# edawson/rkmh

Hardware: AMD Instinct MI355X
Metric: reads classified/sec (higher is better)
Workload: dtype u64; 1 GPU; stream (C2): 1000000 synthetic 150 bp reads per GPU vs data/all_pave_ref.fa (182 refs), k=16 s=1000; reads_per_gpu=1000000, read_len=150, k=16, sketch_size=1000, references=182, parallelism=reads sharded over 1 rank(s); ref sketches RCCL-broadcast once

## Files before the change

rkmh_amd/csrc/rk_kmer.hip:

```cpp
#include "rk_kernels.hpp"

#include <cstdlib>
#include <type_traits>

namespace rk {

namespace {

constexpr int KW = 64;
constexpr int KM_MAX_T = 8;
constexpr int KM_MQ = 32;
constexpr int KM_CH = 2;
constexpr int KM_QCAP = 64 + 4 * KW;
constexpr int KM_LDS_SMALL = 5120;
constexpr int KM_LDS_BIG = 20480;
constexpr int KM_WAVES = 8;

enum { CM_DENSE8 = 0, CM_DENSE16 = 1, CM_SPARSE = 2 };

struct KmerGeom {
    int32_t T;
    int32_t cwords;
    int32_t dset;
    int32_t xcd;
    int32_t nmin_cap;
    int32_t L;
    int32_t gpr[KM_MAX_KS];
    uint32_t magic[KM_MAX_KS];
};

typedef uint32_t u32x4 __attribute__((ext_vector_type(4)));
struct __attribute__((packed, aligned(1))) km_pair1 { uint32_t x, y; };
struct __attribute__((packed, aligned(4))) km_pair4 { uint32_t x, y; };

template <int NQ>
struct KmLds {
    static constexpr int PK = 0;
    static constexpr int INV = PK + NQ * 64 + 2;
    static constexpr int Q = INV + NQ * 32 + 2;
    static constexpr int MQ = Q + KM_QCAP;
    static constexpr int RI = MQ + 2 * KM_MQ;
    static constexpr int NZ = RI + 4 * (KM_MAX_T + 1);
    static constexpr int BEST = NZ + KM_MAX_T;
    static constexpr int FLAGS = BEST + KM_MAX_T;
    static constexpr int NWT = FLAGS + KM_MAX_T;
    static constexpr int FAM = NWT + KM_MAX_T;
    static constexpr int FAMF = FAM + 4 * KM_MAX_T;
    static constexpr int CNT = FAMF + KM_MAX_T;
    static_assert(RI % 4 == 0, "rinfo is read with 16-byte LDS loads");
    static_assert(CNT % 4 == 0, "the multisets are cleared with 16-byte LDS stores");
};
inline size_t km_lds_bytes(const KmerGeom& g, int nq) {
    return ((size_t)(nq == 1 ? KmLds<1>::CNT : KmLds<2>::CNT) + (size_t)g.T * (size_t)(g.cwords + g.dset)) * 4;
}

__device__ __forceinline__ void wave_sync() {
    __builtin_amdgcn_fence(__ATOMIC_RELEASE, "wavefront");
    __builtin_amdgcn_wave_barrier();
    __builtin_amdgcn_fence(__ATOMIC_ACQUIRE, "wavefront");
}
template <int CTRL>
__device__ __forceinline__ int dpp_i32(int v) { return __builtin_amdgcn_update_dpp(v, v, CTRL, 0xf, 0xf, false); }
__device__ __forceinline__ int row_max_i32(int v) {
    int t;
    t = dpp_i32<0xB1>(v); v = t > v ? t : v;
    t = dpp_i32<0x4E>(v); v = t > v ? t : v;
    t = dpp_i32<0x141>(v); v = t > v ? t : v;
    t = dpp_i32<0x140>(v); v = t > v ? t : v;
    return v;
}
__device__ __forceinline__ int half_row_max_i32(int v) {
    int t;
    t = dpp_i32<0xB1>(v); v = t > v ? t : v;
    t = dpp_i32<0x4E>(v); v = t > v ? t : v;
    t = dpp_i32<0x141>(v); v = t > v ? t : v;
    return v;
}

__device__ __forceinline__ uint32_t km_pack4_hi(uint32_t x, uint32_t& mism) {
    const uint32_t c = (x >> 1) & 0x03030303u;
    mism |= (x & 0xDFDFDFDFu) ^ __builtin_amdgcn_perm(0x47544341u, 0x47544341u, c);
    return c * 0x01041040u;
}
__device__ __forceinline__ uint32_t km_pack16(const u32x4& v, uint32_t& mism) {
    const uint32_t m0 = km_pack4_hi(v.x, mism), m1 = km_pack4_hi(v.y, mism), m2 = km_pack4_hi(v.z, mism), m3 = km_pack4_hi(v.w, mism);
    const uint32_t lo = __builtin_amdgcn_perm(m1, m0, 0x0c0c0703u);
    const uint32_t hi = __builtin_amdgcn_perm(m3, m2, 0x07030c0cu);
    return lo | hi;
}
__device__ __forceinline__ uint32_t km_nonzero4(uint32_t m) {
    const uint32_t y = (m | ((m & 0x7f7f7f7fu) + 0x7f7f7f7fu)) & 0x80808080u;
    return ((y >> 7) * 0x01020408u) >> 24;
}

template <int CMODE>
__device__ __forceinline__ uint32_t km_field_max(uint32_t x) {
    if constexpr (CMODE == CM_DENSE8) {
        const uint32_t m01 = max(x & 0xFFu, (x >> 8) & 0xFFu), m23 = max((x >> 16) & 0xFFu, x >> 24);
        return max(m01, m23);
    } else return max(x & 0xFFFFu, x >> 16);
}

template <int KT, int NQ, int CMODE, bool BIG, bool FAM>
__global__ __launch_bounds__(KW, BIG ? 2 : KM_WAVES) void k_classify_kmer(const uint8_t* __restrict__ bases, const uint32_t* __restrict__ offs,
                                                                              uint32_t nreads, int S, RefIndex ix, KmerSets ksets,
                                                                              int32_t* __restrict__ out4, DevPolicy pol, KmerGeom geo) {
    static_assert(KT == 0 || KT == 32 || (KT >= 4 && KT <= 16), "a k-mer packs into 32 bits; the core is the (k-3)-mer");
    constexpr bool WIDE = KT == 32;
    using L = KmLds<NQ>;
    __shared__ __attribute__((aligned(16))) uint32_t smem[(BIG ? KM_LDS_BIG : KM_LDS_SMALL) / 4];
    constexpr uint32_t PAD_P = NQ * 1024;
    constexpr uint32_t clg = CMODE == CM_DENSE8 ? 2 : 1, cbits = 32u >> clg, cmask = (1u << cbits) - 1u;
    uint32_t* const pk = smem + L::PK;
    uint32_t* const inv = smem + L::INV;
    uint32_t* const q = smem + L::Q;
    uint32_t* const mq = smem + L::MQ;
    uint4* const rinfo = reinterpret_cast<uint4*>(smem + L::RI);
    uint32_t* const nzero = smem + L::NZ;
    uint32_t* const best = smem + L::BEST;
    uint32_t* const flags = smem + L::FLAGS;
    uint32_t* const nwtot = smem + L::NWT;
    uint32_t* const fam = smem + L::FAM;
    uint32_t* const famf = smem + L::FAMF;
    uint32_t* const cnt = smem + L::CNT;
    const int T = geo.T;
    const uint32_t CW = (uint32_t)geo.cwords, DS = (uint32_t)geo.dset;
    uint32_t* const dset = cnt + (uint32_t)T * CW;
    const uint32_t ds_shift = 32u - (uint32_t)__builtin_ctz(DS);
    const int lane = threadIdx.x;

    for (uint32_t i = lane; i < ((uint32_t)T * CW) >> 2; i += KW) reinterpret_cast<uint4*>(cnt)[i] = make_uint4(0u, 0u, 0u, 0u);
    const uint32_t ntiles = (nreads + (uint32_t)T - 1) / (uint32_t)T;
    const uintptr_t gb = reinterpret_cast<uintptr_t>(bases);
    const uintptr_t safe_hi = (gb + (uintptr_t)offs[nreads] + 4u) & ~(uintptr_t)3;

    auto tile_reads = [&](uint32_t tl) -> int {
        const uint32_t r = tl * (uint32_t)T;
        return (int)((nreads - r) < (uint32_t)T ? (nreads - r) : (uint32_t)T);
    };
    auto load_offsets = [&](uint32_t tl, uint32_t& a_, uint32_t& b_, uint32_t& o_) {
        const uint32_t r = tl * (uint32_t)T;
        const int n = tile_reads(tl);
        a_ = offs[r];
        b_ = offs[r + (uint32_t)n];
        o_ = offs[r + (uint32_t)(lane <= n ? lane : n)];
    };
    u32x4 pf[NQ];
    auto fetch_tile = [&](uint32_t a_, uint32_t b_) {
        const uintptr_t first = gb + a_;
        const uintptr_t base16 = first & ~(uintptr_t)15;
        const uint32_t nbytes = (uint32_t)(first - base16) + (b_ - a_);
        uint32_t nq = (nbytes + 15u) >> 4;
        if (nq > (uint32_t)(NQ * KW)) nq = NQ * KW;
        const bool safe = base16 >= gb && base16 + 16u * (uintptr_t)nq <= safe_hi;
#pragma unroll
        for (int r = 0; r < NQ; ++r) {
            const uint32_t qi = (uint32_t)r * KW + (uint32_t)lane;
            u32x4 v = {0u, 0u, 0u, 0u};
            if (qi < nq) {
                const uintptr_t qa = base16 + 16u * (uintptr_t)qi;
                if (safe) {
                    typedef const u32x4 __attribute__((address_space(1))) * gq_t;
                    v = __builtin_nontemporal_load((gq_t)qa);
                }
                else {
                    uint32_t d[4];
#pragma unroll
                    for (int j = 0; j < 4; ++j) {
                        const uintptr_t da = qa + 4u * (uintptr_t)j;
                        d[j] = (da >= gb && da + 4u <= safe_hi) ? *reinterpret_cast<const uint32_t*>(da) : 0u;
                    }
                    v.x = d[0]; v.y = d[1]; v.z = d[2]; v.w = d[3];
                }
            }
            pf[r] = v;
        }
    };

    uint32_t tile = blockIdx.x;
    if (geo.xcd) { const uint32_t per = (gridDim.x + 7u) >> 3; tile = (blockIdx.x & 7u) * per + (blockIdx.x >> 3); }
    if (tile >= ntiles) return;
    uint32_t cur_a = 0, cur_b = 0, cur_o = 0;
    load_offsets(tile, cur_a, cur_b, cur_o);
    fetch_tile(cur_a, cur_b);
    {
        const uint32_t r0 = tile * (uint32_t)T;
        const uint32_t ta = (uint32_t)__builtin_amdgcn_readfirstlane((int)cur_a);
        const uint32_t tb = (uint32_t)__builtin_amdgcn_readfirstlane((int)cur_b);
        const uint32_t mis = (uint32_t)((gb + ta) & 15u);
        const uint32_t nbytes = mis + (tb - ta);
        const uint32_t o_next = (uint32_t)__shfl_down((int)cur_o, 1);
        const uint32_t len = o_next - cur_o;
        int Tn = tile_reads(tile);
        uint32_t nq = (nbytes + 15u) >> 4;
        if (nbytes > (uint32_t)(NQ * 1024)) {
            const int Tn0 = Tn;
            Tn = __popcll(__ballot(lane < Tn0 && o_next - ta + mis <= (uint32_t)(NQ * 1024)));
            if (lane >= Tn && lane < Tn0) reinterpret_cast<int4*>(out4)[r0 + lane] = make_int4(-2, 0, 0, 0);
            nq = NQ * KW;
        }

        constexpr int NKC = KT ? 1 : KM_MAX_KS;
        const int NK = KT ? 1 : ksets.n;
        uint32_t nw_all = 0;
        if (lane < Tn) {
#pragma unroll
            for (int j = 0; j < NKC; ++j) if (j < NK) nw_all += (uint32_t)num_windows((int)len, WIDE ? (int)ix.kpk : (KT ? KT : ksets.k[j]), pol.drop_last_window);
        }
        if constexpr (FAM) { if (lane < 4 * KM_MAX_T) fam[lane] = 0; }
        if (lane < KM_MAX_T) {
            nzero[lane] = 0; best[lane] = 0; nwtot[lane] = nw_all;
            if constexpr (FAM) famf[lane] = 0;
            flags[lane] = nw_all > (CMODE == CM_SPARSE ? 0x7FFu : cmask) ? 1u : 0u;
        }
        const uint32_t ulen = (uint32_t)__builtin_amdgcn_readfirstlane((int)len);
        const bool same_len = __ballot(lane < Tn && len != ulen) == 0ull;
        uint32_t mism = 0;
#pragma unroll
        for (int r = 0; r < NQ; ++r) {
            const uint32_t qi = (uint32_t)r * KW + (uint32_t)lane;
            uint32_t m = 0;
            pk[qi] = km_pack16(pf[r], m);
            if (qi < nq) mism |= m;
        }
        if (lane < 2) pk[NQ * KW + lane] = 0;
        const bool has_invalid = __ballot(mism != 0u) != 0ull;
        if (has_invalid) {
#pragma unroll
            for (int r = 0; r < NQ; ++r) {
                const uint32_t qi = (uint32_t)r * KW + (uint32_t)lane;
                uint32_t m0 = 0, m1 = 0, m2 = 0, m3 = 0;
                km_pack4_hi(pf[r].x, m0); km_pack4_hi(pf[r].y, m1); km_pack4_hi(pf[r].z, m2); km_pack4_hi(pf[r].w, m3);
                const uint32_t b16 = km_nonzero4(m0) | (km_nonzero4(m1) << 4) | (km_nonzero4(m2) << 8) | (km_nonzero4(m3) << 12);
                reinterpret_cast<uint16_t*>(inv)[qi] = (uint16_t)(qi < nq ? b16 : 0u);
            }
            if (lane < 2) inv[NQ * 32 + lane] = 0;
        }
        for (int kk = 0; kk < NK; ++kk) {
        const int k = WIDE ? (int)ix.kpk : (KT ? KT : ksets.k[kk]);
        const uint32_t KMASK = (WIDE || k == 16) ? 0xffffffffu : ((1u << (2 * k)) - 1u);
        const uint32_t CMASK = WIDE ? 0xffffffffu : (1u << (2 * (k - 3))) - 1u;
        const uint64_t KMASK64 = WIDE ? (1ull << (2 * k)) - 1ull : 0ull, CMASK64 = WIDE ? (1ull << (2 * (k - 3))) - 1ull : 0ull;
        const uint32_t KBITS = (1u << k) - 1u;
        const uint4* const kf4p = KT ? ix.kf4 : ksets.kf4[kk];
        const uint4* const km1p = KT ? ix.km1 : ksets.km1[kk];
        const uint32_t* const km1v = KT ? ix.km1_vals : ksets.km1_vals[kk];
        const uint32_t kf4_n = KT ? ix.kf4_n : ksets.kf4_n[kk], km1_b = KT ? ix.km1_b : ksets.km1_b[kk];
        wave_sync();
        uint32_t nw = 0, ng = 0;
        if (lane < Tn) { nw = (uint32_t)num_windows((int)len, k, pol.drop_last_window); ng = (nw + 3u) >> 2; }
        uint32_t gs = ng;
        gs += (uint32_t)__builtin_amdgcn_update_dpp(0, (int)gs, 0x111, 0xf, 0xf, true);
        gs += (uint32_t)__builtin_amdgcn_update_dpp(0, (int)gs, 0x112, 0xf, 0xf, true);
        gs += (uint32_t)__builtin_amdgcn_update_dpp(0, (int)gs, 0x114, 0xf, 0xf, true);
        const uint32_t NG = (uint32_t)__builtin_amdgcn_readlane((int)gs, KM_MAX_T - 1);
        if (lane <= KM_MAX_T) rinfo[lane] = make_uint4(cur_o - ta + mis, nw, gs - ng, 0u);
        {
            uint4* d4 = reinterpret_cast<uint4*>(dset);
            for (uint32_t i = lane; i < ((uint32_t)Tn * DS) >> 2; i += KW) d4[i] = make_uint4(0u, 0u, 0u, 0u);
        }
        wave_sync();

        const uint32_t nw_u = (uint32_t)num_windows((int)ulen, k, pol.drop_last_window), gpr_u = (nw_u + 3u) >> 2;
        const bool uniform = same_len && gpr_u >= 2u;
        uint32_t magic = 0;
        if (uniform) magic = ulen == (uint32_t)geo.L ? geo.magic[kk] : (uint32_t)__builtin_amdgcn_readfirstlane((int)(0xFFFFFFFFu / gpr_u + 1u));
        uint32_t magic_v = magic, dlen_v = ulen - 4u * gpr_u;
        asm volatile("" : "+v"(magic_v), "+v"(dlen_v));

        auto count_posting = [&](uint32_t t, uint32_t crow_b, uint32_t ref) -> uint32_t {
            uint32_t* crow = reinterpret_cast<uint32_t*>(reinterpret_cast<uint8_t*>(cnt) + crow_b);
            const uint32_t M1 = CW - 1u, key = ref + 1u;
            uint32_t idx = ((ref * 0x9E3779B1u) >> 16) & M1, probe = 0, c = 0;
            for (; probe <= M1; ++probe) {
                const uint32_t old = atomicCAS(&crow[idx], 0u, (key << 11) | 1u);
                if (old == 0u) { c = 1u; break; }
                if ((old >> 11) == key) { c = (atomicAdd(&crow[idx], 1u) & 0x7FFu) + 1u; break; }
                idx = (idx + 1u) & M1;
            }
            if (probe > M1) { flags[t] = 1; return 0u; }
            return (c << 16) + (0xFFFFu - ref);
        };
        auto add_posting = [&](uint32_t t, uint32_t crow_b, uint32_t ref) {
            if constexpr (CMODE == CM_SPARSE) {
                const uint32_t v = count_posting(t, crow_b, ref);
                if (v) atomicMax(&best[t], v);
            } else {
                const uint32_t sh = (ref << (5 - clg)) & (32u - cbits);
                const uint32_t woff = (ref >> clg) << 2;
                atomicAdd(reinterpret_cast<uint32_t*>(reinterpret_cast<uint8_t*>(cnt) + crow_b + woff), 1u << sh);
            }
        };
        uint32_t mqn = 0;
        auto process_mq = [&]() {
            wave_sync();
            const uint32_t g = (uint32_t)lane >> 4, sl = (uint32_t)lane & 15u;
            auto walk = [&](uint32_t tr, const uint32_t* lp, uint32_t hdr, const km_pair4& pm0) {
                const uint32_t t = tr & 0xFFu, n = hdr & 0xFFFFFFu, base = FAM ? hdr >> 24 : 0u;
                if (base) {
                    if ((tr >> 8) != 0u) return;
                    if (sl == 0) { atomicAdd(&fam[4u * t + ((base - 1u) >> 1)], 1u << (16u * ((base - 1u) & 1u))); famf[t] = 1u; }
                    for (uint32_t c0 = 0; c0 < n; c0 += 16) {
                        const uint32_t c = c0 + sl;
                        if (c < n) {
                            km_pair4 pm = pm0;
                            if (c0) pm = *reinterpret_cast<const km_pair4*>(lp + 1 + 2 * c);
                            const uint32_t sh = (pm.x << (5 - clg)) & (32u - cbits), woff = (pm.x >> clg) << 2;
                            atomicAdd(reinterpret_cast<uint32_t*>(reinterpret_cast<uint8_t*>(cnt) + __umul24(t, CW * 4u) + woff), (pm.y >> 31) ? 0u - (1u << sh) : 1u << sh);
                        }
                    }
                    return;
                }
                for (uint32_t c0 = 0; c0 < n; c0 += 16) {
                    const uint32_t c = c0 + sl;
                    uint32_t v = 0;
                    if (c < n) {
                        km_pair4 pm = pm0;
                        if (c0) pm = *reinterpret_cast<const km_pair4*>(lp + 1 + 2 * c);
                        if ((tr >> 8) < pm.y) {
                            if constexpr (CMODE == CM_SPARSE) v = count_posting(t, __umul24(t, CW * 4u), pm.x);
                            else add_posting(t, __umul24(t, CW * 4u), pm.x);
                        }
                    }
                    if constexpr (CMODE == CM_SPARSE) {
                        v = (uint32_t)row_max_i32((int)v);
                        if (sl == 0 && v) atomicMax(&best[t], v);
                    }
                }
            };
            uint32_t j = g;
            uint32_t tr = 0, n = 0;
            const uint32_t* lp = ix.kpost;
            km_pair4 pm0{0u, 0u};
            if (j < mqn) { tr = mq[2 * j]; lp = ix.kpost + mq[2 * j + 1]; n = lp[0]; pm0 = *reinterpret_cast<const km_pair4*>(lp + 1 + 2 * sl); }
            while (j < mqn) {
                const uint32_t jn = j + KW / 16;
                uint32_t trn = 0, nn = 0;
                const uint32_t* lpn = ix.kpost;
                km_pair4 pmn{0u, 0u};
                if (jn < mqn) { trn = mq[2 * jn]; lpn = ix.kpost + mq[2 * jn + 1]; nn = lpn[0]; pmn = *reinterpret_cast<const km_pair4*>(lpn + 1 + 2 * sl); }
                walk(tr, lp, n, pm0);
                j = jn; tr = trn; lp = lpn; n = nn; pm0 = pmn;
            }
            wave_sync();
            mqn = 0;
        };
        struct Cand { uint32_t key, t, y, key_hi; uint4 c; };
        const uint32_t km_r = WIDE ? 8u : 2u * (uint32_t)k - km1_b, km_vb1 = 32u - KM1_HB - km_r;
        const uint32_t km_vmask = (1u << (km_vb1 - 1u)) - 1u, km_rmask = (1u << km_r) - 1u, nref = (uint32_t)ix.nref;
        auto wide_probe = [&](const Cand& c, const uint4& b, uint32_t hop, uint3& res, bool& again) {
            const uint32_t want = (hop << KW_TAG) | (c.y & ((1u << KW_TAG) - 1u));
            const uint32_t cells[4] = {b.x, b.y, b.z, b.w};
            res = make_uint3(KW_VID_NONE, 0u, 0u);
#pragma unroll
            for (int q = 0; q < 4; ++q) {
                const uint32_t num = cells[q] & KW_EMPTY;
                if ((cells[q] >> (KW_IDBITS + 1)) == want && num != KW_EMPTY && res.x == KW_VID_NONE) {
                    const uint2 kk = ix.kkeys[num];
                    if (kk.x == c.key && (kk.y & 0xFFu) == c.key_hi) res = make_uint3(kk.y >> 8, 0u, num);
                }
            }
            again = res.x == KW_VID_NONE && ((b.w >> KW_IDBITS) & 1u) != 0u && c.t != 0xFFFFFFFFu;
        };
        auto lookup = [&](uint32_t e, uint32_t qn) -> Cand {
            Cand c;
            uint32_t ent = PAD_P | (8u << 12);
            if (e < qn) ent = q[e];
            const uint32_t P = ent & 4095u, t = ent >> 12;
            const km_pair1 w = *reinterpret_cast<const km_pair1*>(reinterpret_cast<const uint8_t*>(pk) + (P >> 2));
            const uint2 ri = *reinterpret_cast<const uint2*>(&rinfo[t]);
            c.t = P - ri.x < ri.y ? t : 0xFFFFFFFFu;
            if constexpr (WIDE) {
                const uint64_t x = (join64(w.x, w.y) >> ((P & 3u) << 1)) & KMASK64;
                const uint64_t r = packed_revcomp64(x, k);
                const uint64_t key = x < r ? x : r;
                c.key = (uint32_t)key; c.key_hi = (uint32_t)(key >> 32);
                c.y = (uint32_t)(kw_y(key, k) >> (2u * (uint32_t)k - km1_b - KW_TAG));
                c.c = km1p[c.y >> KW_TAG];
                return c;
            }
            const uint32_t x = __builtin_amdgcn_alignbit(w.y, w.x, (P & 3u) << 1) & KMASK;
            const uint32_t r = packed_revcomp(x, k);
            c.key = x < r ? x : r;
            c.key_hi = 0;
            c.y = km1_y(c.key, k);
            c.c = km1p[c.y >> km_r];
            return c;
        };
        auto match_cell = [&](const uint4& b, uint32_t wantsh) -> uint32_t {
            const uint32_t lim = 1u << km_vb1;
            return (b.x ^ wantsh) < lim ? b.x : ((b.y ^ wantsh) < lim ? b.y : ((b.z ^ wantsh) < lim ? b.z : ((b.w ^ wantsh) < lim ? b.w : 0xFFFFFFFFu)));
        };
        auto first_match = [&](const Cand& c, uint32_t& cell, bool& again) {
            cell = match_cell(c.c, (c.y & km_rmask) << km_vb1);
            again = (cell & km_vmask) == km_vmask && ((c.c.w >> (km_vb1 - 1u)) & 1u) != 0u && c.t != 0xFFFFFFFFu;
        };
        auto hop_load = [&](const Cand& c, uint32_t hop, bool again) -> u32x4 {
            u32x4 v = {0u, 0u, 0u, 0u};
            if (again) v = *reinterpret_cast<const u32x4*>(km1p + (((c.y >> km_r) + hop) & ((1u << km1_b) - 1u)));
            return v;
        };
        auto next_match = [&](const Cand& c, uint32_t hop, const u32x4& nv, uint32_t& cell, bool& again) {
            if (again) {
                const uint4 nb = make_uint4(nv.x, nv.y, nv.z, nv.w);
                cell = match_cell(nb, ((c.y & km_rmask) << km_vb1) | (hop << (32u - KM1_HB)));
                again = (cell & km_vmask) == km_vmask && ((nb.w >> (km_vb1 - 1u)) & 1u) != 0u;
            }
        };
        auto apply = [&](const Cand& c, uint32_t cell, uint3 wres = make_uint3(0u, 0u, 0u)) {
            uint32_t vid = cell & km_vmask;
            bool hit = vid != km_vmask && c.t != 0xFFFFFFFFu;
            bool zero = vid == km_vmask - 1u;
            if constexpr (WIDE) {
                vid = wres.x;
                hit = vid != KW_VID_NONE && c.t != 0xFFFFFFFFu;
                zero = vid == KW_VID_ZERO;
                if (hit && !zero && ix.keepkey) { const uint32_t kid = ix.kslots[wres.z]; if (!((ix.keepkey[kid >> 5] >> (kid & 31u)) & 1u)) zero = true; }
            }
            uint32_t val = vid | (1u << 20);
            uint32_t valy = 0, valz = 0, valw = 0;
            if (hit && vid >= nref && !zero) {
                const uint4 vv = *reinterpret_cast<const uint4*>(km1v + 4u * (vid - nref));
                val = vv.x; valy = vv.y; valz = vv.z; valw = vv.w;
                if constexpr (CMODE == CM_SPARSE) { if ((val >> 29) == 7u) val = 0x80000000u | valz; }
            }
            uint32_t rank = 0;
            bool multi = false;
            if (hit) {
                if (zero) atomicAdd(&nzero[c.t], 1u);
                else {
                    uint32_t* ds = dset + c.t * DS;
                    const uint32_t id = (WIDE ? wres.z : c.key) + 1u;
                    uint32_t idx = ((id - 1u) * 0x9E3779B1u) >> ds_shift;
                    uint32_t old = atomicCAS(&ds[idx], 0u, id);
                    uint32_t probes = 1;
                    while (old != 0u && probes < DS) {
                        rank += old == id ? 1u : 0u;
                        idx = (idx + 1u) & (DS - 1u);
                        old = atomicCAS(&ds[idx], 0u, id);
                        ++probes;
                    }
                    if (old != 0u) flags[c.t] = 1;
                    else if (FAM && (val >> 29) == 7u) {
                        if (rank == 0) {
                            const uint32_t base = (val >> 26) & 7u, nex = (val >> 22) & 15u, crow_b = __umul24(c.t, CW * 4u);
                            atomicAdd(&fam[4u * c.t + (base >> 1)], 1u << (16u * (base & 1u)));
                            famf[c.t] = 1u;
                            auto signed_add = [&](uint32_t f) {
                                const uint32_t ref = f & 511u, sh = (ref << (5 - clg)) & (32u - cbits);
                                atomicAdd(reinterpret_cast<uint32_t*>(reinterpret_cast<uint8_t*>(cnt) + crow_b + ((ref >> clg) << 2)), (f & 512u) ? 0u - (1u << sh) : 1u << sh);
                            };
                            if (nex > 0u) signed_add(val & 1023u);
                            if (nex > 1u) signed_add((val >> 10) & 1023u);
                            if (nex > 2u) signed_add(valy & 1023u);
                            if (nex > 3u) signed_add((valy >> 10) & 1023u);
                            if (nex > 4u) signed_add((valy >> 20) & 1023u);
                            if (nex > 5u) signed_add(valw & 1023u);
                            if (nex > 6u) signed_add((valw >> 10) & 1023u);
                            if (nex > 7u) signed_add((valw >> 20) & 1023u);
                        }
                    }
                    else if ((val >> 30) == 3u || !(val >> 31)) {
                        const bool three = (val >> 30) == 3u, two = !three && ((val >> 29) & 3u) != 0u;
                        const uint32_t fw = three ? 9u : 11u;
                        const uint32_t lim = (three || two) ? 1u : ((val >> 20) & 0x1FFu);
                        const uint32_t n = rank >= lim ? 0u : (three ? 3u + ((val >> 27) & 3u) : (two ? 2u : 1u));
                        const uint32_t refs[6] = {__builtin_amdgcn_ubfe(val, 0u, three ? 9u : (two ? 11u : 20u)), __builtin_amdgcn_ubfe(val, fw, fw),
                                                  (val >> 18) & 511u, valy & 511u, (valy >> 9) & 511u, (valy >> 18) & 511u};
                        const uint32_t crow_b = __umul24(c.t, CW * 4u);
#pragma unroll
                        for (uint32_t j = 0; j < 6u; ++j) if (j < n) add_posting(c.t, crow_b, refs[j]);
                    } else multi = true;
                }
            }
            const uint32_t listoff = (CMODE == CM_SPARSE ? valz : val) & 0x3fffffffu;
            uint64_t mm = __ballot(multi);
            while (mm) {
                const uint32_t pos = __builtin_amdgcn_mbcnt_hi((uint32_t)(mm >> 32), __builtin_amdgcn_mbcnt_lo((uint32_t)mm, 0u));
                const uint32_t space = (uint32_t)KM_MQ - mqn;
                if (multi && pos < space) {
                    mq[2 * (mqn + pos)] = c.t | (rank << 8); mq[2 * (mqn + pos) + 1] = listoff;
                    multi = false;
                }
                const uint32_t tot = (uint32_t)__popcll(mm);
                mqn += tot < space ? tot : space;
                if (mqn == (uint32_t)KM_MQ) process_mq();
                mm = __ballot(multi);
            }
        };
        auto drain = [&](uint32_t qn) {
            for (uint32_t e0 = 0; e0 < qn; e0 += 2 * KW) {
                const bool two = e0 + KW < qn;
                const Cand a = lookup(e0 + (uint32_t)lane, qn);
                Cand b{0u, 0xFFFFFFFFu, 0u, 0u, make_uint4(0u, 0u, 0u, 0u)};
                if (two) b = lookup(e0 + KW + (uint32_t)lane, qn);
                if constexpr (WIDE) {
                    uint3 ra, rb = make_uint3(KW_VID_NONE, 0u, 0u);
                    bool ga, gb = false;
                    wide_probe(a, a.c, 0u, ra, ga);
                    if (two) wide_probe(b, b.c, 0u, rb, gb);
                    for (uint32_t hop = 1; hop < (1u << KM1_HB) && __ballot(ga || gb); ++hop) {
                        const uint32_t bm = (1u << km1_b) - 1u;
                        if (ga) { const uint4 nb = km1p[((a.y >> KW_TAG) + hop) & bm]; wide_probe(a, nb, hop, ra, ga); }
                        if (gb) { const uint4 nb = km1p[((b.y >> KW_TAG) + hop) & bm]; wide_probe(b, nb, hop, rb, gb); }
                    }
                    apply(a, 0u, ra);
                    if (two) apply(b, 0u, rb);
                    continue;
                }
                uint32_t ca, cb = 0xFFFFFFFFu;
                bool ga, gb = false;
                first_match(a, ca, ga);
                if (two) first_match(b, cb, gb);
                for (uint32_t hop = 1; hop < (1u << KM1_HB) && __ballot(ga || gb); ++hop) {
                    u32x4 na = hop_load(a, hop, ga), nb = hop_load(b, hop, gb);
                    asm volatile("" : "+v"(na), "+v"(nb));
                    next_match(a, hop, na, ca, ga);
                    next_match(b, hop, nb, cb, gb);
                }
                apply(a, ca);
                if (two) apply(b, cb);
            }
            if (mqn) process_mq();
        };

        const uint32_t nsteps = (NG + KW - 1) / KW;
        const bool qlast = !WIDE && NG != 0u && ((NG - 1u) & (uint32_t)(KW - 1)) < 16u;
        const uint32_t kf4_n16 = kf4_n << 4;
        uint32_t qcount = 0;
        uint32_t step = 0;
        for (;;) {
            uint32_t wl[KM_CH], wh[KM_CH], e0v[KM_CH], fq[KM_CH];
            u32x4 fw[KM_CH];
            bool isqv[KM_CH];
#pragma unroll
            for (int s = 0; s < KM_CH; ++s) {
                const bool isq = qlast && step + (uint32_t)s + 1u == nsteps;
                isqv[s] = isq;
                const uint32_t jq = isq ? (uint32_t)lane & 3u : 0u;
                const uint32_t G = (step + (uint32_t)s) * KW + (isq ? (uint32_t)lane >> 2 : (uint32_t)lane);
                uint32_t t, P0;
                if (uniform) {
                    t = __umulhi(G, magic_v);
                    P0 = __umul24(t, dlen_v) + ((G << 2) + mis);
                } else {
                    t = 0;
#pragma unroll
                    for (int i = 1; i < KM_MAX_T; ++i) t += G >= rinfo[i].z ? 1u : 0u;
                    const uint4 ri = rinfo[t];
                    P0 = ri.x + 4u * (G - ri.z);
                }
                const bool act = G < NG;
                if (!act) { P0 = PAD_P; t = 8u; }
                const km_pair1 w = *reinterpret_cast<const km_pair1*>(reinterpret_cast<const uint8_t*>(pk) + (P0 >> 2));
                const uint32_t sh = (P0 & 3u) << 1;
                wl[s] = __builtin_amdgcn_alignbit(w.y, w.x, sh);
                wh[s] = w.y >> sh;
                uint32_t core = k == 16 ? wl[s] >> 6 : (wl[s] >> 6) & CMASK;
                if constexpr (WIDE) core = kw_fold((join64(wl[s], wh[s]) >> 6) & CMASK64);
                const uint32_t sect_b = __umulhi(core * 0x85EBCA6Bu, kf4_n16) & ~15u;
                e0v[s] = P0 | (t << 12);
                fq[s] = 0u;
                fw[s] = u32x4{0u, 0u, 0u, 0u};
                if (isq) {
                    wl[s] = __builtin_amdgcn_alignbit(wh[s], wl[s], 2u * jq);
                    if (act) e0v[s] += jq;
                    fq[s] = *reinterpret_cast<const uint32_t*>(reinterpret_cast<const uint8_t*>(kf4p) + (sect_b + 4u * jq));
                } else fw[s] = *reinterpret_cast<const u32x4*>(reinterpret_cast<const uint8_t*>(kf4p) + sect_b);
            }
            bool stop = false;
            uint32_t done = 0;
            auto test_step = [&](int s, auto inv_tag, auto nw_tag) {
                constexpr bool INV = decltype(inv_tag)::value;
                constexpr int NW = decltype(nw_tag)::value;
                uint32_t ib = 0, nz = 0, nwt = 0, t_ = 0, o0 = 0;
                bool act = true;
                if constexpr (INV) {
                    const uint32_t P0 = e0v[s] & 4095u;
                    t_ = e0v[s] >> 12;
                    act = t_ != 8u;
                    if (act) {
                        ib = __builtin_amdgcn_alignbit(inv[(P0 >> 5) + 1], inv[P0 >> 5], P0 & 31u);
                        const uint2 ri = *reinterpret_cast<const uint2*>(&rinfo[t_]);
                        nwt = ri.y; o0 = P0 - ri.x;
                    }
                }
#pragma unroll
                for (int j = 0; j < NW; ++j) {
                    uint32_t x = j == 0 ? wl[s] : __builtin_amdgcn_alignbit(wh[s], wl[s], 2 * j);
                    if (k < 16) x &= KMASK;
                    if constexpr (WIDE) x = kw_fold((join64(wl[s], wh[s]) >> (2 * j)) & KMASK64);
                    const uint32_t f = NW == 1 ? fq[s] : (j == 0 ? fw[s].x : (j == 1 ? fw[s].y : (j == 2 ? fw[s].z : fw[s].w)));
                    const uint32_t fb = kf4_bits_dev(x);
                    bool cand = (fb & f) == fb;
                    if constexpr (INV) {
                        if (act && ((ib >> j) & KBITS) != 0u) {
                            cand = false;
                            if (o0 + (uint32_t)j < nwt) ++nz;
                        }
                    }
                    const uint64_t m = __builtin_amdgcn_ballot_w64(cand);
                    if (__builtin_amdgcn_inverse_ballot_w64(m)) {
                        const uint32_t mb = __builtin_amdgcn_mbcnt_hi((uint32_t)(m >> 32), __builtin_amdgcn_mbcnt_lo((uint32_t)m, 0u));
                        *reinterpret_cast<uint32_t*>(reinterpret_cast<uint8_t*>(q) + ((mb << 2) + (qcount << 2))) = e0v[s] + (uint32_t)j;
                    }
                    qcount += (uint32_t)__builtin_popcountll(m);
                }
                if constexpr (INV) { if (nz) atomicAdd(&nzero[t_], nz); }
            };
#pragma unroll
            for (int s = 0; s < KM_CH; ++s) {
                if (step + (uint32_t)s < nsteps && !stop) {
                    if (qcount + 4u * KW > (uint32_t)KM_QCAP) stop = true;
                    else {
                        ++done;
                        if (isqv[s]) {
                            if (has_invalid) test_step(s, std::true_type{}, std::integral_constant<int, 1>{});
                            else test_step(s, std::false_type{}, std::integral_constant<int, 1>{});
                        } else if (has_invalid) test_step(s, std::true_type{}, std::integral_constant<int, 4>{});
                        else test_step(s, std::false_type{}, std::integral_constant<int, 4>{});
                    }
                }
            }
            step += done;
            const bool last = step >= nsteps;
            wave_sync();
            const uint32_t qn = last ? qcount : (qcount & ~(uint32_t)(KW - 1));
            drain(qn);
            wave_sync();
            if (last) break;
            const uint32_t rem = qcount - qn;
            uint32_t ce = 0;
            if ((uint32_t)lane < rem) ce = q[qn + lane];
            wave_sync();
            if ((uint32_t)lane < rem) q[lane] = ce;
            qcount = rem;
            wave_sync();
        }

        }
        wave_sync();

        {
            const int lsh = Tn > 4 ? 3 : 4, LPR = 1 << lsh;
            const int g = lane >> lsh, sl = lane & (LPR - 1);
            for (int t = g; t < Tn; t += KW >> lsh) {
                uint32_t* ct = cnt + (uint32_t)t * CW;
                const int nmins = (int)nwtot[t] - (int)nzero[t];
                const bool reroute = nmins > S || flags[t] != 0;
                if (reroute) {
                    if (sl == 0) reinterpret_cast<int4*>(out4)[r0 + t] = make_int4(-2, 0, 0, 0);
                    continue;
                }
                if constexpr (FAM && CMODE != CM_SPARSE) {
                    if (famf[t]) {
                        for (uint32_t b = 0; b < 8u; ++b) {
                            const uint32_t h = (fam[4u * (uint32_t)t + (b >> 1)] >> (16u * (b & 1u))) & 0xFFFFu;
                            if (h == 0u) continue;
                            const uint32_t start = ix.kbase[2u * b], nm = ix.kbase[2u * b + 1u];
                            for (uint32_t m0 = 0; m0 < nm; m0 += (uint32_t)LPR) {
                                const uint32_t m = m0 + (uint32_t)sl;
                                if (m < nm) {
                                    const uint32_t ref = ix.kbase[start + m];
                                    atomicAdd(&ct[ref >> clg], h << ((ref << (5 - clg)) & (32u - cbits)));
                                }
                            }
                        }
                        __builtin_amdgcn_fence(__ATOMIC_RELEASE, "wavefront");
                        __builtin_amdgcn_fence(__ATOMIC_ACQUIRE, "wavefront");
                    }
                }
                int max_id, max_shared, prev;
                if constexpr (CMODE == CM_SPARSE) {
                    const uint32_t bk = best[t];
                    max_id = bk ? (int)(0xFFFFu - (bk & 0xFFFFu)) : 0;
                    max_shared = (int)(bk >> 16);
                    prev = max_id > 0 ? 0 : -1;
                    for (uint32_t w = sl; w < CW; w += LPR) {
                        const uint32_t x = ct[w];
                        const int r_ = (int)(x >> 11) - 1, cj = (int)(x & 0x7FFu);
                        if (x != 0u && r_ < max_id && cj > prev) prev = cj;
                    }
                } else {
                    const uint32_t nwl = (CW + (uint32_t)LPR - 1u) >> lsh, wbase = (uint32_t)sl * nwl;
                    uint32_t lmax = 0, lpre = 0, lfirst = wbase;
                    for (uint32_t i = 0; i < nwl; ++i) {
                        const uint32_t w = wbase + i;
                        const uint32_t m = km_field_max<CMODE>(ct[w < CW ? w : CW - 1u]);
                        if (m > lmax) { lpre = lmax; lmax = m; lfirst = w; }
                    }
                    const uint32_t lkey = (lmax << 8) | (255u - lfirst);
                    const uint32_t km = (uint32_t)(LPR == 16 ? row_max_i32((int)lkey) : half_row_max_i32((int)lkey));
                    const uint32_t M = km >> 8, wb = 255u - (km & 255u);
                    const uint32_t xb = ct[wb];
                    const uint32_t ones = CMODE == CM_DENSE8 ? 0x01010101u : 0x00010001u;
                    const uint32_t y = xb ^ (M * ones);
                    const uint32_t z = (y - ones) & ~y & (ones << (cbits - 1u));
                    const uint32_t qf = (uint32_t)__builtin_ctz(z) >> (5 - clg);
                    max_id = M ? (int)((wb << clg) + qf) : 0;
                    max_shared = (int)M;
                    uint32_t acc = km_field_max<CMODE>(__builtin_amdgcn_ubfe(xb, 0u, qf << (5 - clg)));
                    if (lkey == km) acc = max(acc, lpre);
                    else if (wbase + nwl <= wb) acc = max(acc, lmax);
                    prev = max_id > 0 ? (int)acc : -1;
                }
                prev = LPR == 16 ? row_max_i32(prev) : half_row_max_i32(prev);
                if (sl == 0) reinterpret_cast<int4*>(out4)[r0 + t] = make_int4(max_id, max_shared, max_shared - prev, nmins < geo.nmin_cap ? nmins : geo.nmin_cap);
            }
        }
    }
}

bool make_kmer_geom(KmerGeom& g, int maxlen, int nref, int expect_hits, int win_total, const int* nw_k, int nk, int nq, int& cmode, bool& big) {
    if (maxlen < 1) maxlen = 1;
    cmode = win_total <= 255 ? CM_DENSE8 : CM_DENSE16;
    const int clg = cmode == CM_DENSE8 ? 2 : 1;
    g.cwords = (nref + (1 << clg) - 1) >> clg;
    if (nref > 0 && g.cwords >= 129) { cmode = CM_SPARSE; g.cwords = 128; }
    g.cwords = (g.cwords + 3) & ~3;
    int ds = 64;
    while (ds < 3 * expect_hits && ds < 1024) ds <<= 1;
    g.dset = ds;
    int T = (nq * 1024 - 15) / maxlen;
    if (T > KM_MAX_T) T = KM_MAX_T;
    if (T < 1) T = 1;
    g.T = T;
    big = false;
    while (g.T > 1 && km_lds_bytes(g, nq) > (size_t)KM_LDS_SMALL) g.T -= 1;
    if (km_lds_bytes(g, nq) > (size_t)KM_LDS_SMALL || 2 * g.T < T) {
        big = true;
        g.T = T;
        while (g.T > 1 && km_lds_bytes(g, nq) > (size_t)KM_LDS_BIG) g.T -= 1;
        if (km_lds_bytes(g, nq) > (size_t)KM_LDS_BIG) return false;
    }
    g.xcd = 1;
    g.L = maxlen;
    for (int j = 0; j < KM_MAX_KS; ++j) {
        g.gpr[j] = j < nk ? (nw_k[j] + 3) >> 2 : 0;
        g.magic[j] = g.gpr[j] >= 2 ? 0xFFFFFFFFu / (uint32_t)g.gpr[j] + 1u : 0u;
    }
    return true;
}

template <int KT>
hipError_t launch_k(int nq, int cmode, bool big, bool fam, dim3 grid, hipStream_t st, const uint8_t* bases, const uint32_t* offs, uint32_t nreads,
                    int S, const RefIndex& ix, const KmerSets& ksets, int32_t* out4, const DevPolicy& pol, const KmerGeom& geo) {
#define RK_KM_GO(NQ, CM, BIG, FAM) hipLaunchKernelGGL((k_classify_kmer<KT, NQ, CM, BIG, FAM>), grid, dim3(KW), 0, st, bases, offs, nreads, S, ix, ksets, out4, pol, geo)
#define RK_KM_CM(NQ, BIG)                                                                                    \
    do {                                                                                                     \
        if (cmode == CM_DENSE8) { if (fam) RK_KM_GO(NQ, CM_DENSE8, BIG, true); else RK_KM_GO(NQ, CM_DENSE8, BIG, false); } \
        else if (cmode == CM_DENSE16) { if (fam) RK_KM_GO(NQ, CM_DENSE16, BIG, true); else RK_KM_GO(NQ, CM_DENSE16, BIG, false); } \
        else RK_KM_GO(NQ, CM_SPARSE, BIG, true);                                                             \
    } while (0)
    if (nq == 1 && !big) RK_KM_CM(1, false);
    else if (nq == 1) RK_KM_CM(1, true);
    else if (!big) RK_KM_CM(2, false);
    else RK_KM_CM(2, true);
#undef RK_KM_CM
#undef RK_KM_GO
    return hipGetLastError();
}

}

bool classify_kmer_supported(int nref, int maxlen, int k) {
    return nref <= 16384 && maxlen <= 2 * 1024 - 15 && k >= KPRE_MIN_K && k <= KW_MAX_K;
}

hipError_t launch_classify_kmer(const uint8_t* bases, const uint32_t* offs, uint32_t nreads, const KmerSets& ksets, int S, const RefIndex& ix,
                                int32_t* out4, const DevPolicy& pol, int maxlen, int expect_hits, hipStream_t st, int nmin_cap) {
    if (nreads == 0) return hipSuccess;
    if (ksets.n < 1 || ksets.n > KM_MAX_KS) return hipErrorInvalidValue;
    const int nq = maxlen <= 1024 - 15 ? 1 : 2;
    int nw_k[KM_MAX_KS] = {0}, win_total = 0;
    for (int j = 0; j < ksets.n; ++j) { nw_k[j] = num_windows(maxlen, ksets.k[j], pol.drop_last_window); win_total += nw_k[j]; }
    KmerGeom geo;
    int cmode = 0;
    bool big = false;
    if (!make_kmer_geom(geo, maxlen, ix.nref, expect_hits, win_total, nw_k, ksets.n, nq, cmode, big)) return hipErrorInvalidConfiguration;
    geo.nmin_cap = nmin_cap;
    const uint32_t ntiles = (nreads + (uint32_t)geo.T - 1) / (uint32_t)geo.T;
    const bool fam = ix.kbase_n != 0u;
    uint32_t grid = ntiles;
    grid = (grid + 7u) & ~7u;
    if (ksets.n > 1) return launch_k<0>(nq, cmode, big, fam, dim3(grid), st, bases, offs, nreads, S, ix, ksets, out4, pol, geo);
#define RK_KM_K(KT) case KT: return launch_k<KT>(nq, cmode, big, fam, dim3(grid), st, bases, offs, nreads, S, ix, ksets, out4, pol, geo)
    switch (ksets.k[0]) {
        RK_KM_K(8); RK_KM_K(9); RK_KM_K(10); RK_KM_K(11); RK_KM_K(12); RK_KM_K(13); RK_KM_K(14); RK_KM_K(15); RK_KM_K(16);
        case 17: case 18: case 19: case 20:
            return ix.kkeys ? launch_k<32>(nq, cmode, big, fam, dim3(grid), st, bases, offs, nreads, S, ix, ksets, out4, pol, geo) : hipErrorInvalidValue;
        default: return hipErrorInvalidValue;
    }
#undef RK_KM_K
}

}
```

Measured before the change: 3.354 billion reads/s.

## Pack candidate queue to 16-bit entries, widen step chunk, defer drains

Candidate queue entries are stored as 16-bit values instead of 32-bit, doubling queue capacity within the same LDS footprint. The step chunk grows from 2 to 4 for narrow k-mer instantiations, and the loop now skips the drain whenever another full step still fits, so drains happen less often and on larger batches. This removes wave syncs and drain overhead per window, at the cost of more live registers for the larger unrolled chunk and reliance on entries fitting in 16 bits.

```diff
diff --git a/rkmh_amd/csrc/rk_kmer.hip b/rkmh_amd/csrc/rk_kmer.hip
--- a/rkmh_amd/csrc/rk_kmer.hip
+++ b/rkmh_amd/csrc/rk_kmer.hip
@@ -10,8 +10,11 @@
 constexpr int KW = 64;
 constexpr int KM_MAX_T = 8;
 constexpr int KM_MQ = 32;
-constexpr int KM_CH = 2;
-constexpr int KM_QCAP = 64 + 4 * KW;
+constexpr int KM_CH = 4;
+constexpr int KM_QDW = 64 + 4 * KW;
+constexpr int KM_QCAP = 2 * KM_QDW;
+static_assert(KM_QCAP * sizeof(uint16_t) == 1280, "the queue keeps its 1280 bytes: the LDS layout behind it, T and 8 waves per SIMD depend on it");
+static_assert(KW - 1 + 4 * KW <= KM_QCAP, "after a mid-tile drain (remainder < 64) the next step always fits: the window loop makes progress");
 constexpr int KM_LDS_SMALL = 5120;
 constexpr int KM_LDS_BIG = 20480;
 constexpr int KM_WAVES = 8;
@@ -38,7 +41,8 @@
     static constexpr int PK = 0;
     static constexpr int INV = PK + NQ * 64 + 2;
     static constexpr int Q = INV + NQ * 32 + 2;
-    static constexpr int MQ = Q + KM_QCAP;
+    static constexpr int MQ = Q + KM_QDW;
+    static_assert(((NQ * 1024 + 3) | (KM_MAX_T << 12)) <= 0xFFFF && NQ * 1024 + 3 < (1 << 12), "a queue entry fits 16 bits: P <= the padding's position + 3, read <= 8");
     static constexpr int RI = MQ + 2 * KM_MQ;
     static constexpr int NZ = RI + 4 * (KM_MAX_T + 1);
     static constexpr int BEST = NZ + KM_MAX_T;
@@ -107,13 +111,14 @@
                                                                               int32_t* __restrict__ out4, DevPolicy pol, KmerGeom geo) {
     static_assert(KT == 0 || KT == 32 || (KT >= 4 && KT <= 16), "a k-mer packs into 32 bits; the core is the (k-3)-mer");
     constexpr bool WIDE = KT == 32;
+    constexpr int CH = (KT == 0 || WIDE) ? 2 : KM_CH;
     using L = KmLds<NQ>;
     __shared__ __attribute__((aligned(16))) uint32_t smem[(BIG ? KM_LDS_BIG : KM_LDS_SMALL) / 4];
     constexpr uint32_t PAD_P = NQ * 1024;
     constexpr uint32_t clg = CMODE == CM_DENSE8 ? 2 : 1, cbits = 32u >> clg, cmask = (1u << cbits) - 1u;
     uint32_t* const pk = smem + L::PK;
     uint32_t* const inv = smem + L::INV;
-    uint32_t* const q = smem + L::Q;
+    uint16_t* const q = reinterpret_cast<uint16_t*>(smem + L::Q);
     uint32_t* const mq = smem + L::MQ;
     uint4* const rinfo = reinterpret_cast<uint4*>(smem + L::RI);
     uint32_t* const nzero = smem + L::NZ;
@@ -530,11 +535,11 @@
         uint32_t qcount = 0;
         uint32_t step = 0;
         for (;;) {
-            uint32_t wl[KM_CH], wh[KM_CH], e0v[KM_CH], fq[KM_CH];
-            u32x4 fw[KM_CH];
-            bool isqv[KM_CH];
-#pragma unroll
-            for (int s = 0; s < KM_CH; ++s) {
+            uint32_t wl[CH], wh[CH], e0v[CH], fq[CH];
+            u32x4 fw[CH];
+            bool isqv[CH];
+#pragma unroll
+            for (int s = 0; s < CH; ++s) {
                 const bool isq = qlast && step + (uint32_t)s + 1u == nsteps;
                 isqv[s] = isq;
                 const uint32_t jq = isq ? (uint32_t)lane & 3u : 0u;
@@ -568,8 +573,6 @@
                     fq[s] = *reinterpret_cast<const uint32_t*>(reinterpret_cast<const uint8_t*>(kf4p) + (sect_b + 4u * jq));
                 } else fw[s] = *reinterpret_cast<const u32x4*>(reinterpret_cast<const uint8_t*>(kf4p) + sect_b);
             }
-            bool stop = false;
-            uint32_t done = 0;
             auto test_step = [&](int s, auto inv_tag, auto nw_tag) {
                 constexpr bool INV = decltype(inv_tag)::value;
                 constexpr int NW = decltype(nw_tag)::value;
@@ -602,35 +605,32 @@
                     const uint64_t m = __builtin_amdgcn_ballot_w64(cand);
                     if (__builtin_amdgcn_inverse_ballot_w64(m)) {
                         const uint32_t mb = __builtin_amdgcn_mbcnt_hi((uint32_t)(m >> 32), __builtin_amdgcn_mbcnt_lo((uint32_t)m, 0u));
-                        *reinterpret_cast<uint32_t*>(reinterpret_cast<uint8_t*>(q) + ((mb << 2) + (qcount << 2))) = e0v[s] + (uint32_t)j;
+                        *reinterpret_cast<uint16_t*>(reinterpret_cast<uint8_t*>(q) + ((mb << 1) + (qcount << 1))) = (uint16_t)(e0v[s] + (uint32_t)j);
                     }
                     qcount += (uint32_t)__builtin_popcountll(m);
                 }
                 if constexpr (INV) { if (nz) atomicAdd(&nzero[t_], nz); }
             };
 #pragma unroll
-            for (int s = 0; s < KM_CH; ++s) {
-                if (step + (uint32_t)s < nsteps && !stop) {
-                    if (qcount + 4u * KW > (uint32_t)KM_QCAP) stop = true;
-                    else {
-                        ++done;
-                        if (isqv[s]) {
-                            if (has_invalid) test_step(s, std::true_type{}, std::integral_constant<int, 1>{});
-                            else test_step(s, std::false_type{}, std::integral_constant<int, 1>{});
-                        } else if (has_invalid) test_step(s, std::true_type{}, std::integral_constant<int, 4>{});
-                        else test_step(s, std::false_type{}, std::integral_constant<int, 4>{});
-                    }
-                }
-            }
-            step += done;
+            for (int s = 0; s < CH; ++s) {
+                if (step < nsteps && qcount + 4u * KW <= (uint32_t)KM_QCAP) {
+                    if (isqv[s]) {
+                        if (has_invalid) test_step(s, std::true_type{}, std::integral_constant<int, 1>{});
+                        else test_step(s, std::false_type{}, std::integral_constant<int, 1>{});
+                    } else if (has_invalid) test_step(s, std::true_type{}, std::integral_constant<int, 4>{});
+                    else test_step(s, std::false_type{}, std::integral_constant<int, 4>{});
+                    ++step;
+                } else break;
+            }
             const bool last = step >= nsteps;
+            if (!last && qcount + 4u * KW <= (uint32_t)KM_QCAP) continue;
             wave_sync();
             const uint32_t qn = last ? qcount : (qcount & ~(uint32_t)(KW - 1));
             drain(qn);
             wave_sync();
             if (last) break;
             const uint32_t rem = qcount - qn;
-            uint32_t ce = 0;
+            uint16_t ce = 0;
             if ((uint32_t)lane < rem) ce = q[qn + lane];
             wave_sync();
             if ((uint32_t)lane < rem) q[lane] = ce;
```

New measurement: 3.425 billion reads/s, median of 6. 2.1% higher.
